# DataArcTech/RAG-ARC

Measured on AMD Instinct MI355X. Metric: queries/sec at fixed (N_corpus, d), exact top-k (ids bit-exact vs CPU oracle), higher is better.
Workload: dtype f16; 1 GPU; 100000000x768 fp16 corpus of N(0,1) directions resident in HBM, row-sharded over 1 GPU(s), batch 256 queries, cosine top-100, exact (canonical fp32 rescore); n_corpus=100000000, d=768, batch=256, k=100, rows_per_gpu=100000000, exchange=none (one shard), repaired_queries_last_step=0

## Files before the change

include/rarc.h:

```cpp
#ifndef RARC_H
#define RARC_H

#include <stddef.h>
#include <stdint.h>

#ifdef __cplusplus
extern "C" {
#endif

#define RARC_VERSION 600

#define RARC_OK 0
#define RARC_E_INVALID -1
#define RARC_E_HIP -2
#define RARC_E_WORKSPACE -3
#define RARC_E_UNSUPPORTED -4
#define RARC_E_IO -5

#define RARC_MAX_QUERIES 256
#define RARC_MAX_K 1024
#define RARC_DIM_ALIGN 128

#define RARC_Q_OK 0u
#define RARC_Q_UNCERTAIN 1u
// ... 231 lines not shown
int rarc_wordpiece_encode(const RarcWordPiece* wp, const char* text_blob, const int64_t* text_offsets, int n_texts,
                          int max_length, int32_t* h_ids, int64_t ld_ids, int32_t* h_lens, int n_threads);

#define RARC_IO_DIRECT 1
#define RARC_IO_FSYNC 2
#define RARC_IO_TRUNCATE 4
typedef struct RarcIoStats {
  int64_t bytes;
  double seconds;
  double file_seconds;
  double copy_wait_seconds;
  int64_t direct_bytes;
  int64_t n_chunks, slot_bytes;
  int n_threads, direct;
} RarcIoStats;
int rarc_file_to_device(const char* path, int n_seg, const int64_t* h_file_off, const int64_t* h_bytes,
                        const int64_t* h_dev_off, void* d_base, int64_t d_capacity_bytes, void* h_staging,
                        size_t staging_bytes, int n_threads, int flags, void* stream, RarcIoStats* stats);
int rarc_device_to_file(const char* path, int n_seg, const int64_t* h_file_off, const int64_t* h_bytes,
                        const int64_t* h_dev_off, const void* d_base, int64_t d_capacity_bytes, void* h_staging,
                        size_t staging_bytes, int n_threads, int flags, void* stream, RarcIoStats* stats);

size_t rarc_wide_workspace_bytes(int d_pad, int cand_cap);
int rarc_search_wide(const void* d_rows, const uint16_t* d_image16, int fmt, int64_t n_rows, int d_pad, float max_norm,
                     float rho, const void* d_qblock, int nq, int k, int64_t id_base, int64_t* d_out_ids,
                     float* d_out_scores, uint32_t* d_status, void* d_ws, size_t ws_bytes, int cand_cap, void* stream);

int rarc_row_sqnorms(const void* d_rows, int fmt, int64_t n_rows, int d_pad, int64_t first_row, float* d_xn, void* stream);
int rarc_search_wide_l2(const void* d_rows, const uint16_t* d_image16, int fmt, int64_t n_rows, int d_pad, float max_norm,
                        float rho, const float* d_xn, const void* d_qblock, int nq, int k, int64_t id_base, int64_t* d_out_ids,
                        float* d_out_scores, uint32_t* d_status, void* d_ws, size_t ws_bytes, int cand_cap, void* stream);
int rarc_debug_wide_bounds(const void* d_ws, size_t ws_bytes, int d_pad, int cand_cap, float* d_out, void* stream);
int rarc_debug_query_scale8(float mx, float* sq, float* qi);

size_t rarc_search_rows_workspace_bytes(int nq, int k);
int rarc_search_rows(const void* d_rows, int fmt, int64_t n_rows, int d_pad, const void* d_qblock, int nq, const int64_t* d_list,
                     int64_t m, int k, int64_t id_base, const float* d_xn, int l2, int64_t* d_out_ids, float* d_out_scores,
                     uint32_t* d_status, void* d_ws, size_t ws_bytes, void* stream);
int rarc_strike_rows(const int64_t* d_ids, const float* d_scores, int nq, int kprime, const uint32_t* d_bits, int64_t n_rows,
                     int64_t id_base, int k, int l2, int64_t* d_out_ids, float* d_out_scores, uint32_t* d_count, void* stream);

size_t rarc_search_rows_grouped_workspace_bytes(int nq, int k);
int rarc_search_rows_grouped(const void* d_rows, int fmt, int64_t n_rows, int d_pad, const void* d_qblock, int nq,
                             const int64_t* d_lists, const int64_t* d_tiles, int n_tiles, int64_t m_max, int k, int64_t id_base,
                             const float* d_xn, int l2, int64_t* d_out_ids, float* d_out_scores, uint32_t* d_status, void* d_ws,
                             size_t ws_bytes, void* stream);
int rarc_strike_rows_grouped(const int64_t* d_ids, const float* d_scores, int nq, int kprime, const uint32_t* d_bits,
                             const int64_t* d_bits_off, int64_t n_rows, int64_t id_base, int k, int l2, int64_t* d_out_ids,
                             float* d_out_scores, uint32_t* d_count, void* stream);

size_t rarc_similar_pairs_workspace_bytes(int64_t n_rows, int d, int cand_cap);
int rarc_similar_pairs(const float* d_rows, int64_t ld, int64_t n_rows, int d, double threshold, void* d_ws, size_t ws_bytes,
                       int cand_cap, int64_t* d_out_pairs, double* d_out_scores, int64_t out_cap,
                       unsigned long long* d_out_count, uint32_t* d_flags, void* stream);

size_t rarc_knn_graph_workspace_bytes(int64_t n_rows, int d, int top_k, int cand_cap);
int rarc_knn_graph(const float* d_rows, int64_t ld, int64_t n_rows, int d, int top_k, double cutoff, void* d_ws, size_t ws_bytes,
                   int cand_cap, int64_t* d_out_ids, double* d_out_scores, int32_t* d_out_count, uint32_t* d_flags, void* stream);

size_t rarc_graph_csr_workspace_bytes(int64_t n, int64_t m);
int rarc_graph_csr(const int64_t* d_pairs, const uint32_t* d_weights, const uint32_t* d_loops, int64_t n, int64_t m, void* d_graph,
                   size_t graph_bytes, void* stream);
size_t rarc_louvain_workspace_bytes(int64_t n, int64_t m);
int rarc_louvain_init(const void* d_graph, size_t graph_bytes, int64_t n, int64_t m, void* d_state, size_t state_bytes, int64_t* d_out3,
                      void* stream);
int rarc_louvain_sweep(const void* d_graph, size_t graph_bytes, int64_t n, int64_t m, void* d_state, size_t state_bytes, int cur, int sweep,
// ... 49 lines not shown
```

rag-arc_amd/csrc/rarc_common.h:

```cpp
#pragma once
#include <hip/hip_runtime.h>
#include <stdint.h>
#include <stddef.h>
#include "../../include/rarc.h"

#if (defined(SCAN_HALFREAD) || defined(RARC_Q8_ABLATIONS) || defined(G256_SKIP_A1)) && !defined(RARC_EXPERIMENT)
#error "SCAN_HALFREAD / RARC_Q8_ABLATIONS / G256_SKIP_A1 build kernels with wrong results: measurement builds only, add -DRARC_EXPERIMENT"
#endif
#ifdef RARC_EXPERIMENT
#define RARC_BUILD_VERSION (RARC_VERSION + 100000)
#else
#define RARC_BUILD_VERSION RARC_VERSION
#endif

typedef _Float16 half_t;
typedef _Float16 half8 __attribute__((ext_vector_type(8)));
typedef float f32x16 __attribute__((ext_vector_type(16)));

#define RARC_GPTR(p) ((const __attribute__((address_space(1))) void*)(p))
#define RARC_LPTR(p) ((__attribute__((address_space(3))) void*)(p))

constexpr int RARC_NB = 256;
constexpr int RARC_MAX_WG = 256;
constexpr int RARC_SEED_TILES = 128;
constexpr int RARC_SEED_MAX_TILES = 2048;
constexpr size_t RARC_WS_THR = 0;
constexpr size_t RARC_WS_BINLO = 1024;
constexpr size_t RARC_WS_BINSCALE = 2048;
constexpr size_t RARC_WS_BININV = 3072;
constexpr size_t RARC_WS_CNT = 4096;
constexpr size_t RARC_WS_FLAGS = 5120;
static_assert(RARC_WS_FLAGS + 4 == RARC_WS_ANYFLAG_OFFSET, "include/rarc.h out of sync");
constexpr size_t RARC_WS_HIST = 8192;
constexpr size_t RARC_WS_CNT2 = RARC_WS_HIST + (size_t)RARC_MAX_QUERIES * RARC_NB * 4;
constexpr size_t RARC_WS_SEED = RARC_WS_CNT2 + (size_t)RARC_MAX_WG * RARC_MAX_QUERIES * 4;
constexpr size_t RARC_WS_CAND = RARC_WS_SEED + (size_t)RARC_MAX_QUERIES * RARC_SEED_MAX_TILES * 32 * 4;

struct RarcWs {
  float* thr;
  float* binlo;
  float* binscale;
  float* bininv;
  uint32_t* cnt;
  uint32_t* flags;
  uint32_t* hist;
  uint32_t* cnt2;
  float* seed;
  uint64_t* cand;
};
static inline RarcWs rarc_ws_carve(void* base) {
  char* b = (char*)base;
  RarcWs w;
  w.thr = (float*)(b + RARC_WS_THR);
  w.binlo = (float*)(b + RARC_WS_BINLO);
  w.binscale = (float*)(b + RARC_WS_BINSCALE);
  w.bininv = (float*)(b + RARC_WS_BININV);
  w.cnt = (uint32_t*)(b + RARC_WS_CNT);
  w.flags = (uint32_t*)(b + RARC_WS_FLAGS);
  w.hist = (uint32_t*)(b + RARC_WS_HIST);
  w.cnt2 = (uint32_t*)(b + RARC_WS_CNT2);
  w.seed = (float*)(b + RARC_WS_SEED);
  w.cand = (uint64_t*)(b + RARC_WS_CAND);
  return w;
}
// ... 263 lines not shown
```

rag-arc_amd/csrc/scan_q8.hip:

```cpp
#include "rarc_common.h"
#include <stdio.h>

struct ScanQ8Params {
  const uint4* corpus;
  const float* tmeta;
  const float* hq;
  const int8_t* q8;
  const float* qinv;
  const float* eps8;
  uint32_t n_rows;
  uint32_t n_tiles;
  uint32_t t_begin;
  uint32_t resume;
  float hot_margin;
  uint32_t* thr;
  const float* binlo;
  const float* binscale;
  const float* bininv;
  uint32_t* hist;
  uint32_t* cnt2;
  uint64_t* cand;
  uint32_t seg;
  uint32_t kprime;
  uint32_t nq;
  unsigned long long* dbg;
};

#ifndef Q8_M16_FP16_ROWS
#define Q8_M16_FP16_ROWS 0
#endif
#ifndef Q8_BIG_PF
#define Q8_BIG_PF 1
#endif
#ifndef Q8_BIG_NG
#define Q8_BIG_NG 2
#endif
#ifndef Q8_EB
#define Q8_EB 0
#endif
constexpr int Q8_WAVES = 8;
constexpr int Q8_THREADS = Q8_WAVES * 64;

constexpr int Q8_WSTAGE = 768;
constexpr int Q8_STAGE = 8 * Q8_WSTAGE;
constexpr int Q8_TB_SLOTS = 16;
constexpr int Q8_TB_STRIDE = 80;

template <bool B>
struct Q8Flag { static constexpr bool value = B; };
constexpr int Q8_DEEP_D = 384;

typedef uint32_t q8_u32x4 __attribute__((ext_vector_type(4)));

template <int D, bool M16V = false>
struct ScanQ8Lds {
  static constexpr int RS = D + (M16V ? 32 : 16);
  static constexpr int TILE = 32 * RS;
  static constexpr int CNT = 2 * TILE;
  static constexpr int BINLO = CNT + 1024;
  static constexpr int BINSCALE = BINLO + 1024;
  static constexpr int BININV = BINSCALE + 1024;
  static constexpr int EPS8 = BININV + 1024;
  static constexpr int HLAND = EPS8 + 1024;
  static constexpr int SKEY = HLAND + 1024;
  static constexpr int SQ = SKEY + 8 * Q8_STAGE;
  static constexpr int TB = (SQ + Q8_STAGE + 15) & ~15;
  static constexpr int TOTAL = TB + Q8_WAVES * Q8_TB_SLOTS * Q8_TB_STRIDE;
};

__device__ __forceinline__ half_t q8_tile_scale(float w) { return __builtin_bit_cast(half_t, (uint16_t)__float_as_uint(w)); }
__device__ __forceinline__ float q8_tile_rt(float w) { return (float)__builtin_bit_cast(half_t, (uint16_t)(__float_as_uint(w) >> 16)); }

__device__ __forceinline__ void q8_lds_barrier() {
  asm volatile("s_waitcnt lgkmcnt(0)\n\ts_barrier" ::: "memory");
}

typedef int q8_i32x16 __attribute__((ext_vector_type(16)));
__device__ __forceinline__ int q8_all16(const q8_i32x16& a) {
  int x = a[0];
#pragma unroll
  for (int i = 1; i < 16; ++i) x ^= a[i];
  return x;
}

template <int D, int FMT = 0, int ABL = 0>
__global__ __launch_bounds__(Q8_THREADS) void rarc_scan_q8_kernel(const ScanQ8Params p) {
  static_assert(D % 128 == 0 && D >= 128 && D <= 1024, "D must be a multiple of 128, <= 1024");
  extern __shared__ __attribute__((aligned(16))) char smem[];
  using L = ScanQ8Lds<D, (FMT != 0) || Q8_M16_FP16_ROWS>;
  constexpr int KS = D / 32;
  static_assert(FMT == 0 || D % 256 == 0, "fp8 rows are padded to a multiple of 256");
  constexpr int EPC = FMT ? 16 : 8;
  constexpr int CPR = D / EPC;
  constexpr int CPT = 32 * CPR / Q8_THREADS;
  constexpr int MSTRIDE = FMT == 1 ? RARC_QMETA_F8_STRIDE : RARC_QMETA_STRIDE;
  constexpr int TCH = 32 * CPR;
  constexpr bool NT_ROWS = !(ABL & 262144);

  const int tid = threadIdx.x;
  const int wave = __builtin_amdgcn_readfirstlane(tid >> 6);
  const int lane = tid & 63;
  const int row = lane & 31, h = lane >> 5;
  constexpr bool M16 = (FMT != 0) || Q8_M16_FP16_ROWS;
  const uint32_t q_lo = wave * 32 + (lane & 15);
  const uint32_t qidx = M16 ? q_lo + 16 * (lane >> 5) : wave * 32 + row;
  const int rq = lane >> 4;
  const int rql = rq & 1;
  auto row_of = [&](uint32_t r) -> uint32_t { return M16 ? (r & 3) + 16 * ((r >> 2) & 1) + 8 * (r >> 3) : (r & 3) + 8 * (r >> 2); };
  const unsigned long long dbg_c0 = p.dbg ? __builtin_amdgcn_s_memtime() : 0ull;
  const unsigned long long dbg_r0 = p.dbg ? __builtin_amdgcn_s_memrealtime() : 0ull;

  uint32_t* s_cnt = (uint32_t*)(smem + L::CNT);
  float* s_binlo = (float*)(smem + L::BINLO);
  float* s_binscale = (float*)(smem + L::BINSCALE);
  float* s_bininv = (float*)(smem + L::BININV);
  float* s_eps8 = (float*)(smem + L::EPS8);
// ... 11 lines not shown

  constexpr int KS2 = D / 64;
  i32x4 qf[KS];
  if constexpr (M16) {
    const int8_t* qp = p.q8 + (size_t)q_lo * D + 16 * rq;
#pragma unroll
    for (int ks = 0; ks < KS2; ++ks) {
      qf[2 * ks] = *(const i32x4*)(qp + 64 * ks);
      qf[2 * ks + 1] = *(const i32x4*)(qp + 16 * D + 64 * ks);
    }
  } else {
    const int8_t* qp = p.q8 + (size_t)qidx * D + 16 * h;
#pragma unroll
    for (int ks = 0; ks < KS; ++ks) qf[ks] = *(const i32x4*)(qp + 32 * ks);
  }
  const float my_qinv = p.qinv[qidx];
  const float my_hq = p.hq[qidx];
  const float r_max = p.tmeta[0 - RARC_QMETA_HDR];
  float thr = __uint_as_float(p.thr[qidx]);
  __builtin_amdgcn_s_waitcnt(0x0F70);

  constexpr bool WOFF_REGS = (D <= 768);
  auto woff_of = [&](int j) {
    const uint32_t c = j * Q8_THREADS + tid;
    return (c / CPR) * L::RS + (c % CPR) * EPC;
  };
  uint32_t woff[WOFF_REGS ? CPT : 1];
  if constexpr (WOFF_REGS) {
#pragma unroll
    for (int j = 0; j < CPT; ++j) woff[j] = woff_of(j);
  }
  const uint32_t aoff = M16 ? (lane & 15) * L::RS + 16 * rq : row * L::RS + 16 * h;

  const uint32_t t0 = p.t_begin + blockIdx.x, stride = gridDim.x;
  const bool has_own = blockIdx.x < p.nq;
  const uint32_t own_q = has_own ? blockIdx.x : 0u;
  const uint32_t* hword = p.hist + (size_t)own_q * RARC_NB + 32 * wave + row;

  struct Fetch {
    uint4 c[CPT];
    float mul[FMT == 1 ? CPT : 1];
    float2 meta;
    uint32_t thr;
    uint32_t hw;
  };
  auto clamp_tile = [&](uint32_t t) { return t < p.n_tiles ? t : 0u; };
  auto fetch = [&](Fetch& f, uint32_t tile, auto refresh) {
    f.meta = *(const float2*)(p.tmeta + (size_t)tile * MSTRIDE);
    if constexpr (FMT == 1) {
#pragma unroll
      for (int j = 0; j < CPT; ++j)
        f.mul[j] = p.tmeta[(size_t)tile * MSTRIDE + 2 + (j * Q8_THREADS + tid) / CPR];
    }
    if constexpr (decltype(refresh)::value) {
      f.thr = __hip_atomic_load(&p.thr[qidx], __ATOMIC_RELAXED, __HIP_MEMORY_SCOPE_AGENT);
      f.hw = __hip_atomic_load(hword, __ATOMIC_RELAXED, __HIP_MEMORY_SCOPE_AGENT);
    }
    __builtin_amdgcn_sched_barrier(0);
    const uint4* src = p.corpus + (size_t)tile * TCH + tid;
#pragma unroll
    for (int j = 0; j < CPT; ++j) {
      if constexpr (NT_ROWS)
        f.c[j] = __builtin_bit_cast(uint4, __builtin_nontemporal_load((const q8_u32x4*)(src + j * Q8_THREADS)));
      else
        f.c[j] = src[j * Q8_THREADS];
    }
  };
  uint32_t opaque_zero = 0;
  asm volatile("" : "+v"(opaque_zero));
  auto convert_chunk = [&](const Fetch& f, int j, half_t s, char* dst) {
    char* at = dst + (WOFF_REGS ? woff[WOFF_REGS ? j : 0] : woff_of(j));
    if constexpr (FMT == 2) {
      const uint4 v = f.c[j];
      *(uint4*)at = make_uint4(v.x ^ opaque_zero, v.y ^ opaque_zero, v.z ^ opaque_zero, v.w ^ opaque_zero);
    } else if constexpr (FMT == 1) {
      if (ABL & 16) {
        const uint4 v = f.c[j];
        *(uint4*)at = make_uint4(v.x ^ opaque_zero, v.y ^ opaque_zero, v.z ^ opaque_zero, v.w ^ opaque_zero);
      } else {
// ... 188 lines not shown
          rs = acc[r] == m ? (uint32_t)r : rs;
        }
      }
      if (__builtin_amdgcn_ballot_w64(c > 1) == 0) {
        const uint32_t doc = row0 + row_of(rs);
        stage_n(pass && doc < p.n_rows, (float)m * sc, doc);
      } else {
#pragma unroll
        for (int r = 0; r < 16; ++r) {
          const float a = (float)acc[r] * sc;
          const uint32_t doc = row0 + row_of((uint32_t)r);
          stage_n(a >= thr && doc < p.n_rows, a, doc);
        }
      }
      }
    }
  };
  auto flush = [&]() __attribute__((always_inline)) {
    drain();
    const uint32_t n = wcount < (uint32_t)Q8_WSTAGE ? wcount : (uint32_t)Q8_WSTAGE;
    for (uint32_t e0 = 0; e0 < n; e0 += 64) {
      const uint32_t e = e0 + lane;
      const bool v = e < n;
      const uint32_t qq = v ? (uint32_t)my_sq[e] : qidx;
      const uint64_t key = v ? my_skey[e] : 0ull;
      const float tcur = __shfl(thr, (int)(M16 ? (qq & 15u) + 2u * (qq & 16u) : (qq & 31u)), 64);
      const bool hot = (ABL & 16384) || rarc_candscore(key) >= tcur + p.hot_margin * s_eps8[qq];
      if (v && rarc_candscore(key) >= tcur) emit(qq, key, hot);
    }
    wcount = 0;
  };

  constexpr int NG = D <= Q8_DEEP_D ? 4 : (FMT != 0 ? (D <= 768 ? 2 : Q8_BIG_NG) : (D <= 896 ? 2 : 1));
  Fetch f[NG];
  fetch(f[0], t0, Q8Flag<true>{});
  convert_tile(f[0], 0);
  float2 mcur[2];
  mcur[0] = f[0].meta;
  __builtin_amdgcn_sched_barrier(0);
  constexpr bool PP = (D <= 768) && !(ABL & 256);
  const bool grp_b = PP && wave >= Q8_WAVES / 2;
  constexpr bool EB = Q8_EB && !PP && !(ABL & 512);
  if constexpr (NG == 4) {
    fetch(f[1], clamp_tile(t0 + stride), Q8Flag<true>{});
    __builtin_amdgcn_sched_barrier(0);
    fetch(f[2], clamp_tile(t0 + 2 * stride), Q8Flag<true>{});
    __builtin_amdgcn_sched_barrier(0);
    fetch(f[3], clamp_tile(t0 + 3 * stride), Q8Flag<true>{});
    __builtin_amdgcn_sched_barrier(0);
    if (!grp_b) fetch(f[0], clamp_tile(t0 + 4 * stride), Q8Flag<true>{});
  } else if constexpr (NG == 2) {
    fetch(f[1], clamp_tile(t0 + stride), Q8Flag<true>{});
    __builtin_amdgcn_sched_barrier(0);
    if (!grp_b) fetch(f[0], clamp_tile(t0 + 2 * stride), Q8Flag<true>{});
  } else {
    fetch(f[0], clamp_tile(t0 + stride), Q8Flag<true>{});
  }
  __builtin_amdgcn_sched_barrier(0);
  float last_pub = has_own ? __uint_as_float(p.thr[own_q]) : -INFINITY;
  __builtin_amdgcn_s_waitcnt(0x0F70);
  q8_lds_barrier();

  i32x16 acc_b = {0};
  bool live_prev = false;
  uint32_t it = 0;
#define Q8_STAMP(slot)                                                                                        \
  if ((ABL & 1024) && blockIdx.x == 0 && it >= 1000 && it < 1016 && lane == 0)                                 \
    p.dbg[8 + ((it - 1000) * Q8_WAVES + wave) * 8 + (slot)] = __builtin_amdgcn_s_memtime();
#define Q8_RF(g) (NG != 4 || (g) == 1)
#define Q8_ITER(PAR, GB, G, GP)                                                                               \
  {                                                                                                           \
    Q8_STAMP(0)                                                                                               \
    if (!(GB)) {             \
      const float tinv = mcur[PAR].y, tsc = mcur[PAR].x;                                                      \
      i32x16 acc;                                                                                             \
      acc = mfma_convert(PAR, f[G]);                                                                  \
      mcur[(PAR) ^ 1] = f[G].meta;                                                                    \
      Q8_STAMP(1)                                                                                             \
      if (!(ABL & 8) && Q8_RF(G)) {                                                                           \
        thr = fmaxf(thr, __uint_as_float(f[G].thr));                                                  \
        if (lane < 32) s_hland[32 * wave + lane] = f[G].hw;                                           \
      }                                                                                                       \
      if constexpr (EB) {                                \
        Q8_STAMP(3)                                                                                           \
        q8_lds_barrier();                                                                                     \
        Q8_STAMP(4)                                                                                           \
      }                                                                                                       \
      if (!(ABL & 1) && live) prune(acc, cur, tinv, tsc);                                                     \
      else if (q8_all16(acc) == 0x7fffffff) p.cnt2[0] = 1;  \
      Q8_STAMP(2)                                                                                             \
                                                                \
      if (!(ABL & 2)) fetch(f[G], clamp_tile(cur + (NG + 1) * stride), Q8Flag<Q8_RF(G)>{});           \
    } else {  \
      if (!(ABL & 1) && live_prev) prune(acc_b, cur - stride, mcur[(PAR) ^ 1].y, mcur[(PAR) ^ 1].x);          \
      live_prev = live;                                                                                       \
      Q8_STAMP(1)                                                                                             \
      if (!(ABL & 2)) fetch(f[GP], clamp_tile(cur + NG * stride), Q8Flag<Q8_RF(GP)>{});                       \
      __builtin_amdgcn_sched_barrier(0);           \
// ... 4 lines not shown
        thr = fmaxf(thr, __uint_as_float(f[G].thr));                                                          \
        if (lane < 32) s_hland[32 * wave + lane] = f[G].hw;                                                   \
      }                                                                                                       \
      if ((ABL & 1) && q8_all16(acc_b) == 0x7fffffff) p.cnt2[0] = 1;                                          \
    }                                                                                                         \
    if constexpr (!EB) {                                                                                      \
      Q8_STAMP(3)                                                                                             \
      q8_lds_barrier();                                                                                       \
      Q8_STAMP(4)                                                                                             \
    }                                                                                                         \
    ++it;                                                                                                     \
                      \
    if (!(ABL & 8) && wave == 0 && has_own && (it <= 16 || (it & 3) == 0)) {                                  \
      const int b = rarc_wave_find_from_top_256(s_hland[4 * lane], s_hland[4 * lane + 1],                     \
                                                s_hland[4 * lane + 2], s_hland[4 * lane + 3], p.kprime);      \
      if (b >= 2 && lane == 0) {                                                                              \
        const float lo = s_binlo[own_q];                                                                      \
        const float t = fmaxf(rarc_bin_threshold(b, lo, s_bininv[own_q]) - 2.0002f * s_eps8[own_q], lo);      \
        if (t > last_pub) {                  \
          last_pub = t;                                                                                       \
          __hip_atomic_store(&p.thr[own_q], __float_as_uint(t), __ATOMIC_RELAXED, __HIP_MEMORY_SCOPE_AGENT);  \
        }                                                                                                     \
      }                                                                                                       \
    }                                                                                                         \
                  \
    if (!(ABL & 64) && (wcount | tb_n) != 0 &&                                                                 \
        (it <= 16 || (it & (it - 1)) == 0 || (it & 127) == 0 || wcount > (uint32_t)Q8_WSTAGE / 2))            \
      flush();                                                                                                \
  }

#define Q8_STEP(OFF, PAR, GB, G, GP)                                                  \
    {                                                                                 \
      const uint32_t cur = base + (OFF) * stride;                                     \
      const bool live = (OFF) == 0 || cur < p.n_tiles;                                \
      Q8_ITER(PAR, GB, G, GP)                                                         \
    }
#define Q8_LOOP(GB)                                                                   \
  if constexpr (NG == 4) {                                                            \
    for (uint32_t base = t0; base < p.n_tiles; base += 4 * stride) {                  \
      Q8_STEP(0, 0, GB, 1, 0) Q8_STEP(1, 1, GB, 2, 1) Q8_STEP(2, 0, GB, 3, 2) Q8_STEP(3, 1, GB, 0, 3) \
    }                                                                                 \
  } else {                                                                            \
    for (uint32_t base = t0; base < p.n_tiles; base += 2 * stride) {                  \
      Q8_STEP(0, 0, GB, NG == 2 ? 1 : 0, 0) Q8_STEP(1, 1, GB, 0, NG == 2 ? 1 : 0)     \
    }                                                                                 \
  }
  if (grp_b) {
    Q8_LOOP(true)
  } else {
    Q8_LOOP(false)
  }
#undef Q8_STEP
#undef Q8_LOOP
#undef Q8_ITER
#undef Q8_RF
  if (grp_b && !(ABL & 1) && live_prev)
    prune(acc_b, t0 + (((p.n_tiles - 1 - t0) / stride) | (NG == 4 ? 3u : 1u)) * stride, mcur[1].y, mcur[1].x);
  flush();
  __syncthreads();
  if (tid < RARC_MAX_QUERIES) p.cnt2[(size_t)blockIdx.x * RARC_MAX_QUERIES + tid] = s_cnt[tid];
  if (p.dbg && blockIdx.x == 0 && tid == 0) {
    p.dbg[0] = __builtin_amdgcn_s_memtime() - dbg_c0;
    p.dbg[1] = __builtin_amdgcn_s_memrealtime() - dbg_r0;
  }
}

bool rarc_prof_next(hipEvent_t* start, hipEvent_t* stop);
int rarc_seed_launch(const void* corpus, const float* rowscale, int fmt, int64_t n_rows, int d_pad,
                     const uint16_t* q16, int nq, int kprime, float bin_lo, float bin_hi, const float* sub_a,
                     const float* sub_b, const RarcWs& ws, hipStream_t s, int64_t rows_covered, const float* floor);
int rarc_scan_f16_stage_launch(const uint16_t* corpus, int64_t n_rows, uint32_t stage_tiles, int d_pad, const uint16_t* q16,
                               const float* eps16, int nq, int kprime, const RarcWs& ws, int cap, int grid, hipStream_t s);

template <int D, int FMT, int ABL = 0>
static int launch_scan_q8(const ScanQ8Params& p, int grid, hipStream_t s) {
  constexpr size_t lds = ScanQ8Lds<D, (FMT != 0) || Q8_M16_FP16_ROWS>::TOTAL;
  static RarcPerDevice attr_done;
  if (size_t& done = attr_done.cur(); !done) {
    RARC_HIP_CHECK(hipFuncSetAttribute((const void*)rarc_scan_q8_kernel<D, FMT, ABL>,
                                       hipFuncAttributeMaxDynamicSharedMemorySize, (int)lds));
    done = 1;
  }
#ifdef RARC_Q8_ABLATIONS
  if constexpr (ABL == 0 && ((D == 1024 && FMT == 1) || (D == 768 && FMT == 0) || (D == 768 && FMT == 2))) {
    static const int abl = getenv("RARC_Q8_ABL") ? atoi(getenv("RARC_Q8_ABL")) : 0;
    if (abl == 262144) return launch_scan_q8<D, FMT, 262144>(p, grid, s);
    if (abl == 262149) return launch_scan_q8<D, FMT, 262149>(p, grid, s);
    if (abl == 1) return launch_scan_q8<D, FMT, 1>(p, grid, s);
    if (abl == 4) return launch_scan_q8<D, FMT, 4>(p, grid, s);
    if (abl == 5) return launch_scan_q8<D, FMT, 5>(p, grid, s);
    if (abl == 9) return launch_scan_q8<D, FMT, 9>(p, grid, s);
    if constexpr (FMT == 1) {
      if (abl == 1024 || abl == 1025) {
        static unsigned long long* d_dbg = nullptr;
        if (!d_dbg) RARC_HIP_CHECK(hipMalloc((void**)&d_dbg, 65536));
        RARC_HIP_CHECK(hipMemsetAsync(d_dbg, 0, 65536, s));
        ScanQ8Params pd = p;
        pd.dbg = d_dbg;
        hipFuncSetAttribute((const void*)rarc_scan_q8_kernel<D, FMT, 1024>, hipFuncAttributeMaxDynamicSharedMemorySize, (int)lds);
        hipFuncSetAttribute((const void*)rarc_scan_q8_kernel<D, FMT, 1025>, hipFuncAttributeMaxDynamicSharedMemorySize, (int)lds);
        if (abl == 1024) hipLaunchKernelGGL((rarc_scan_q8_kernel<D, FMT, 1024>), dim3(grid), dim3(Q8_THREADS), lds, s, pd);
        else hipLaunchKernelGGL((rarc_scan_q8_kernel<D, FMT, 1025>), dim3(grid), dim3(Q8_THREADS), lds, s, pd);
        RARC_HIP_CHECK(hipStreamSynchronize(s));
        if (const char* path = getenv("RARC_Q8_TIMELINE"); path && p.n_tiles - p.t_begin > 1100u * (uint32_t)grid) {
          static unsigned long long h[8192];
          RARC_HIP_CHECK(hipMemcpy(h, d_dbg, 65536, hipMemcpyDeviceToHost));
          if (FILE* f = fopen(path, "a")) {
            fprintf(f, "launch tiles [%u, %u) abl %d: per iteration and wave, shader cycles relative to wave 0's start of the iteration: start | after mfma+convert | after prune | after fetch issue | after barrier\n", p.t_begin, p.n_tiles, abl);
            for (int it = 2; it < 10; ++it)
              for (int w = 0; w < Q8_WAVES; ++w) {
                const unsigned long long* r = &h[8 + (it * Q8_WAVES + w) * 8];
                const unsigned long long b0 = h[8 + (it * Q8_WAVES) * 8];
                fprintf(f, "it %2d w%d: %6lld %6lld %6lld %6lld %6lld   (next iteration starts at %lld)\n", it, w, (long long)(r[0] - b0), (long long)(r[1] - b0),
                        (long long)(r[2] - b0), (long long)(r[3] - b0), (long long)(r[4] - b0), (long long)(h[8 + ((it + 1) * Q8_WAVES + w) * 8] - b0));
              }
            fclose(f);
          }
        }
// ... 41 lines not shown
                 FMTV == 0 ? 128 : 256);
  return RARC_E_UNSUPPORTED;
}

int rarc_scan_q8_launch(const void* corpus, const float* rowscale, int fmt, int64_t n_rows, int d_pad,
                        const float* qmeta, const uint16_t* q16, const int8_t* q8, const float* qinv,
                        const float* eps16, const float* eps8, int nq, int kprime, float bin_lo, float bin_hi,
                        const RarcWs& ws, int cap, int* grid_out, hipStream_t s, const int8_t* shadow8,
                        int (*tighten)(void* ctx, int n_wg, int mode), void* tighten_ctx, const float* hq, const float* floor,
                        int* hybrid_out) {
  ScanQ8Params p;
  p.hq = hq;
  p.corpus = fmt == 2 ? (const uint4*)shadow8 : (const uint4*)corpus;
  p.tmeta = qmeta + RARC_QMETA_HDR;
  p.q8 = q8;
  p.qinv = qinv;
  p.eps8 = eps8;
  p.n_rows = (uint32_t)n_rows;
  p.n_tiles = (uint32_t)((n_rows + 31) / 32);
  p.t_begin = 0;
  p.resume = 0;
  p.hot_margin = 1.0f;
  p.thr = (uint32_t*)ws.thr;
  p.binlo = ws.binlo;
  p.binscale = ws.binscale;
  p.bininv = ws.bininv;
  p.hist = ws.hist;
  p.cnt2 = ws.cnt2;
  p.cand = ws.cand;
  p.seg = (uint32_t)(cap / RARC_MAX_WG);
  p.kprime = (uint32_t)kprime;
  p.nq = (uint32_t)nq;
  p.dbg = nullptr;

  int dev = 0, cus = 256;
  RARC_HIP_CHECK(hipGetDevice(&dev));
  RARC_HIP_CHECK(hipDeviceGetAttribute(&cus, hipDeviceAttributeMultiprocessorCount, dev));
  int grid = cus < RARC_MAX_WG ? cus : RARC_MAX_WG;
  if (const char* e = getenv("RARC_SCAN_Q8_WGS")) { const int g = atoi(e); if (g >= 8 && g < grid) grid = g; }
  if ((uint32_t)grid > p.n_tiles) grid = (int)p.n_tiles;
  *grid_out = grid;
  auto launch = [&](const ScanQ8Params& pp) {
    return fmt == 2 ? dispatch_scan_q8<2>(pp, d_pad, grid, s)
                    : fmt == 1 ? dispatch_scan_q8<1>(pp, d_pad, grid, s) : dispatch_scan_q8<0>(pp, d_pad, grid, s);
  };
  static const int split_mode = getenv("RARC_SCAN_SPLIT") ? atoi(getenv("RARC_SCAN_SPLIT")) : 3;
  const uint32_t pair = 2u * (uint32_t)(grid > 0 ? grid : 1);
  uint32_t cuts[3];
  int n_cuts = 0;
  if (tighten && split_mode > 0) {
    uint32_t div[3] = {512u, 64u, 8u};
    if (const char* e = getenv("RARC_SPLIT_DIVS")) {
      unsigned a = 0, b = 0, c = 0;
      const int got = sscanf(e, "%u,%u,%u", &a, &b, &c);
      if (got >= 1) { div[0] = a; div[1] = got >= 2 ? b : 0; div[2] = got >= 3 ? c : 0; }
    }
    for (int i = (split_mode >= 3 ? 0 : (split_mode == 2 ? 1 : 2)); i < 3; ++i) {
      if (div[i] == 0) continue;
      const uint32_t t = (p.n_tiles / div[i]) / pair * pair;
      static const int min_env = getenv("RARC_SPLIT_MIN") ? atoi(getenv("RARC_SPLIT_MIN")) : 0;
      const uint32_t min_pairs = min_env > 0 ? (uint32_t)min_env : (div[i] == 8u ? 16u : 8u);
      if (t >= min_pairs * pair && (n_cuts == 0 || t > cuts[n_cuts - 1])) cuts[n_cuts++] = t;
    }
  }
  int rc = rarc_seed_launch(corpus, rowscale, fmt == 2 ? 0 : fmt, n_rows, d_pad, q16, nq, kprime, bin_lo, bin_hi, eps16,
                            eps8, ws, s, n_cuts ? (int64_t)cuts[0] * 32 : 0, floor);
  if (rc) return rc;
  if (p.n_tiles == 0) return RARC_OK;
  RARC_REQUIRE(rarc_gate_scan(s) == 0, RARC_E_HIP, "rarc_scan_q8: hipStreamWaitEvent on the gate event failed");
  uint32_t begin = 0;
  static const int hybrid_env = getenv("RARC_HYBRID") ? atoi(getenv("RARC_HYBRID")) : 1;
  static const int hybrid_div = getenv("RARC_HYBRID_DIV") ? atoi(getenv("RARC_HYBRID_DIV")) : 8;
  if (hybrid_out) *hybrid_out = 0;
  if (hybrid_out && hybrid_env && tighten && fmt == 0 && d_pad <= 768 && n_cuts == 0 && hybrid_div >= 2) {
    const uint32_t stage = (p.n_tiles / (uint32_t)hybrid_div) / pair * pair;
    if (stage >= 2u * pair && stage < p.n_tiles) {
      if ((rc = rarc_scan_f16_stage_launch((const uint16_t*)corpus, n_rows, stage, d_pad, q16, eps16, nq, kprime, ws, cap, grid,
                                           s)) != RARC_OK)
        return rc;
      if ((rc = tighten(tighten_ctx, grid, 2)) != RARC_OK) return rc;
      ScanQ8Params pi = p;
      pi.t_begin = stage;
      pi.resume = 1u;
      pi.hot_margin = 0.f;
      *hybrid_out = 1;
      return launch(pi);
    }
  }
  for (int i = 0; i <= n_cuts; ++i) {
    ScanQ8Params pi = p;
    pi.t_begin = begin;
    pi.n_tiles = i < n_cuts ? cuts[i] : p.n_tiles;
    pi.resume = i > 0 ? 1u : 0u;
    pi.hot_margin = i > 0 ? 0.f : 1.0f;
    if ((rc = launch(pi)) != RARC_OK) return rc;
    if (i < n_cuts && (rc = tighten(tighten_ctx, grid, 1)) != RARC_OK) return rc;
    begin = pi.n_tiles;
  }
  return RARC_OK;
}
```

rag-arc_amd/hip/binding.py:

```python
from __future__ import annotations

import ctypes
import os
import threading
from ctypes import c_double, c_float, c_int, c_int64, c_size_t, c_uint64, c_void_p

_PKG = os.path.dirname(os.path.dirname(os.path.abspath(__file__)))
_LIB = os.environ.get("RARC_LIBRARY") or os.path.join(_PKG, "lib", "librarc_hip.so")

MAX_QUERIES = 256
MAX_K = 1024
WIDE_MAX_K = 8192
WIDE_MAX_DPAD = 4096
DIM_ALIGN = 128
Q_UNCERTAIN = 1
Q_OVERFLOW = 2
WS_ANYFLAG_OFFSET = 5124


class RarcError(RuntimeError):
    """Raised for every non-zero status returned by librarc_hip.so."""


class RarcUnsupported(RarcError, NotImplementedError):
# ... 140 lines not shown
    "rarc_enc32_gemm": (c_int, [c_void_p, c_void_p, c_void_p, c_void_p, c_void_p, c_void_p, c_int, c_int, c_int, c_void_p]),
    "rarc_enc32_workspace_bytes": (c_size_t, [c_int, c_int, c_int]),
    "rarc_enc32_forward": (c_int, [c_void_p, c_void_p, c_void_p, c_int, c_int, c_int, c_void_p, c_size_t, c_void_p,
                                   c_void_p]),
    "rarc_lm_workspace_bytes": (c_size_t, [c_void_p, c_int]),
    "rarc_lm_yes_no_logits": (c_int, [c_void_p, c_void_p, c_void_p, c_int, c_int, c_int, c_int, c_void_p, c_size_t, c_void_p,
                                      c_void_p]),
    "rarc_lm_prefix_cache_bytes": (c_size_t, [c_void_p, c_int]),
    "rarc_lm_prefix_kv": (c_int, [c_void_p, c_void_p, c_void_p, c_int, c_int, c_void_p, c_size_t, c_void_p, c_size_t, c_void_p]),
    "rarc_lm_yes_no_logits_prefixed": (c_int, [c_void_p, c_void_p, c_void_p, c_int, c_int, c_void_p, c_void_p, c_int, c_int,
                                                c_void_p, c_int, c_int, c_void_p, c_size_t, c_void_p, c_void_p]),
    "rarc_lm_embed_last": (c_int, [c_void_p, c_void_p, c_void_p, c_int, c_int, c_int, c_int, c_void_p, c_size_t, c_void_p, c_int64,
                                   c_void_p]),
    "rarc_lm_embed_last_prefixed": (c_int, [c_void_p, c_void_p, c_void_p, c_int, c_int, c_void_p, c_void_p, c_int, c_int, c_void_p,
                                            c_int, c_int, c_void_p, c_size_t, c_void_p, c_int64, c_void_p]),
    "rarc_wordpiece_create": (c_int, [ctypes.c_char_p, c_size_t, c_int, ctypes.c_char_p, ctypes.c_char_p, ctypes.c_char_p,
                                      ctypes.c_char_p, ctypes.c_char_p, c_size_t, c_int, ctypes.POINTER(c_void_p)]),
    "rarc_wordpiece_destroy": (None, [c_void_p]),
    "rarc_wordpiece_encode": (c_int, [c_void_p, ctypes.c_char_p, c_void_p, c_int, c_int, c_void_p, c_int64, c_void_p, c_int]),
    "rarc_file_to_device": (c_int, [ctypes.c_char_p, c_int, ctypes.POINTER(c_int64), ctypes.POINTER(c_int64),
                                    ctypes.POINTER(c_int64), c_void_p, c_int64, c_void_p, c_size_t, c_int, c_int, c_void_p,
                                    ctypes.POINTER(IoStats)]),
    "rarc_device_to_file": (c_int, [ctypes.c_char_p, c_int, ctypes.POINTER(c_int64), ctypes.POINTER(c_int64),
                                    ctypes.POINTER(c_int64), c_void_p, c_int64, c_void_p, c_size_t, c_int, c_int, c_void_p,
                                    ctypes.POINTER(IoStats)]),
    "rarc_wide_workspace_bytes": (c_size_t, [c_int, c_int]),
    "rarc_search_wide": (c_int, [c_void_p, c_void_p, c_int, c_int64, c_int, c_float, c_float, c_void_p, c_int, c_int, c_int64,
                                 c_void_p, c_void_p, c_void_p, c_void_p, c_size_t, c_int, c_void_p]),
    "rarc_row_sqnorms": (c_int, [c_void_p, c_int, c_int64, c_int, c_int64, c_void_p, c_void_p]),
    "rarc_search_wide_l2": (c_int, [c_void_p, c_void_p, c_int, c_int64, c_int, c_float, c_float, c_void_p, c_void_p, c_int, c_int,
                                    c_int64, c_void_p, c_void_p, c_void_p, c_void_p, c_size_t, c_int, c_void_p]),
    "rarc_debug_wide_bounds": (c_int, [c_void_p, c_size_t, c_int, c_int, c_void_p, c_void_p]),
    "rarc_debug_query_scale8": (c_int, [c_float, ctypes.POINTER(c_float), ctypes.POINTER(c_float)]),
    "rarc_search_rows_workspace_bytes": (c_size_t, [c_int, c_int]),
    "rarc_search_rows": (c_int, [c_void_p, c_int, c_int64, c_int, c_void_p, c_int, c_void_p, c_int64, c_int, c_int64, c_void_p, c_int,
                                 c_void_p, c_void_p, c_void_p, c_void_p, c_size_t, c_void_p]),
    "rarc_strike_rows": (c_int, [c_void_p, c_void_p, c_int, c_int, c_void_p, c_int64, c_int64, c_int, c_int, c_void_p, c_void_p,
                                 c_void_p, c_void_p]),
    "rarc_search_rows_grouped_workspace_bytes": (c_size_t, [c_int, c_int]),
    "rarc_search_rows_grouped": (c_int, [c_void_p, c_int, c_int64, c_int, c_void_p, c_int, c_void_p, c_void_p, c_int, c_int64, c_int,
                                         c_int64, c_void_p, c_int, c_void_p, c_void_p, c_void_p, c_void_p, c_size_t, c_void_p]),
    "rarc_strike_rows_grouped": (c_int, [c_void_p, c_void_p, c_int, c_int, c_void_p, c_void_p, c_int64, c_int64, c_int, c_int,
                                         c_void_p, c_void_p, c_void_p, c_void_p]),
    "rarc_similar_pairs_workspace_bytes": (c_size_t, [c_int64, c_int, c_int]),
    "rarc_similar_pairs": (c_int, [c_void_p, c_int64, c_int64, c_int, ctypes.c_double, c_void_p, c_size_t, c_int, c_void_p, c_void_p,
                                   c_int64, c_void_p, c_void_p, c_void_p]),
    "rarc_knn_graph_workspace_bytes": (c_size_t, [c_int64, c_int, c_int, c_int]),
    "rarc_knn_graph": (c_int, [c_void_p, c_int64, c_int64, c_int, c_int, ctypes.c_double, c_void_p, c_size_t, c_int, c_void_p, c_void_p,
                               c_void_p, c_void_p, c_void_p]),
    "rarc_graph_csr_workspace_bytes": (c_size_t, [c_int64, c_int64]),
    "rarc_graph_csr": (c_int, [c_void_p, c_void_p, c_void_p, c_int64, c_int64, c_void_p, c_size_t, c_void_p]),
    "rarc_louvain_workspace_bytes": (c_size_t, [c_int64, c_int64]),
    "rarc_louvain_init": (c_int, [c_void_p, c_size_t, c_int64, c_int64, c_void_p, c_size_t, c_void_p, c_void_p]),
    "rarc_louvain_sweep": (c_int, [c_void_p, c_size_t, c_int64, c_int64, c_void_p, c_size_t, c_int, c_int, c_void_p, c_void_p]),
    "rarc_louvain_aggregate": (c_int, [c_void_p, c_size_t, c_int64, c_int64, c_void_p, c_size_t, c_int, c_void_p, c_int64, c_void_p,
                                       c_void_p, c_void_p, c_void_p, c_void_p]),
    "rarc_louvain_labels_workspace_bytes": (c_size_t, [c_int64]),
    "rarc_louvain_labels": (c_int, [c_void_p, c_int64, c_void_p, c_size_t, c_void_p]),
    "rarc_louvain_limits": (c_int, [ctypes.POINTER(c_int)]),
    "rarc_ppr_workspace_bytes": (c_size_t, [c_int64, c_int64, c_int]),
    "rarc_ppr_seed": (c_int, [c_void_p, c_size_t, c_int64, c_int64, c_void_p, c_void_p, c_int, c_int, c_void_p, c_size_t, c_void_p]),
    "rarc_ppr_step": (c_int, [c_void_p, c_size_t, c_int64, c_int64, c_int, c_int, c_int64, c_int, c_void_p, c_size_t, c_void_p,
                              c_void_p]),
    "rarc_ppr_scores": (c_int, [c_int64, c_int64, c_int, c_void_p, c_size_t, c_void_p, c_void_p]),
    "rarc_ppr_topk": (c_int, [c_int64, c_int64, c_int, c_int, c_int, c_void_p, c_size_t, c_void_p, c_void_p, c_void_p, c_void_p]),
    "rarc_ppr_limits": (c_int, [ctypes.POINTER(c_int)]),
# ... 59 lines not shown
```

Before: 9480 queries/s.

## Add dynamic tail scheduling with guided chunk claims to q8 scan

```diff
diff --git a/include/rarc.h b/include/rarc.h
--- a/include/rarc.h
+++ b/include/rarc.h
@@ -287,6 +287,11 @@
                         float* d_out_scores, uint32_t* d_status, void* d_ws, size_t ws_bytes, int cand_cap, void* stream);
 int rarc_debug_wide_bounds(const void* d_ws, size_t ws_bytes, int d_pad, int cand_cap, float* d_out, void* stream);
 int rarc_debug_query_scale8(float mx, float* sq, float* qi);
+int rarc_debug_q8_tail_plan(uint32_t t_begin, uint32_t n_tiles, uint32_t grid, int d_pad, int fmt, int pct, int min_mib,
+                            uint32_t* t_dyn, uint32_t* r0, uint32_t* unit);
+int rarc_debug_q8_tail_chunks(uint32_t k_first, uint32_t n, uint32_t stride, uint32_t unit, uint32_t t_dyn, uint32_t r0,
+                              uint32_t n_tiles, uint32_t* t0, uint32_t* t_end);
+int64_t rarc_debug_q8_tail_counter_offset(int launch);
 
 size_t rarc_search_rows_workspace_bytes(int nq, int k);
 int rarc_search_rows(const void* d_rows, int fmt, int64_t n_rows, int d_pad, const void* d_qblock, int nq, const int64_t* d_list,
diff --git a/rag-arc_amd/csrc/rarc_common.h b/rag-arc_amd/csrc/rarc_common.h
--- a/rag-arc_amd/csrc/rarc_common.h
+++ b/rag-arc_amd/csrc/rarc_common.h
@@ -30,6 +30,7 @@
 constexpr size_t RARC_WS_BININV = 3072;
 constexpr size_t RARC_WS_CNT = 4096;
 constexpr size_t RARC_WS_FLAGS = 5120;
+constexpr int RARC_WS_TAIL_FLAG = 32;
 static_assert(RARC_WS_FLAGS + 4 == RARC_WS_ANYFLAG_OFFSET, "include/rarc.h out of sync");
 constexpr size_t RARC_WS_HIST = 8192;
 constexpr size_t RARC_WS_CNT2 = RARC_WS_HIST + (size_t)RARC_MAX_QUERIES * RARC_NB * 4;
diff --git a/rag-arc_amd/csrc/scan_q8.hip b/rag-arc_amd/csrc/scan_q8.hip
--- a/rag-arc_amd/csrc/scan_q8.hip
+++ b/rag-arc_amd/csrc/scan_q8.hip
@@ -1,5 +1,8 @@
 #include "rarc_common.h"
 #include <stdio.h>
+#ifdef RARC_Q8_ABLATIONS
+#include <algorithm>
+#endif
 
 struct ScanQ8Params {
   const uint4* corpus;
@@ -23,6 +26,9 @@
   uint32_t seg;
   uint32_t kprime;
   uint32_t nq;
+  uint32_t t_dyn;
+  uint32_t tail_r0;
+  uint32_t* tail_ctr;
   unsigned long long* dbg;
 };
 
@@ -45,6 +51,9 @@
 constexpr int Q8_STAGE = 8 * Q8_WSTAGE;
 constexpr int Q8_TB_SLOTS = 16;
 constexpr int Q8_TB_STRIDE = 80;
+constexpr int Q8_DBG_BYTES = 65536;
+constexpr int Q8_FIN_SLOT = 2048;
+static_assert((Q8_FIN_SLOT + 2 * RARC_MAX_WG) * 8 <= Q8_DBG_BYTES, "finish stamps past the debug buffer");
 
 template <bool B>
 struct Q8Flag { static constexpr bool value = B; };
@@ -65,7 +74,8 @@
   static constexpr int SKEY = HLAND + 1024;
   static constexpr int SQ = SKEY + 8 * Q8_STAGE;
   static constexpr int TB = (SQ + Q8_STAGE + 15) & ~15;
-  static constexpr int TOTAL = TB + Q8_WAVES * Q8_TB_SLOTS * Q8_TB_STRIDE;
+  static constexpr int TICK = TB + Q8_WAVES * Q8_TB_SLOTS * Q8_TB_STRIDE;
+  static constexpr int TOTAL = TICK + 16;
 };
 
 __device__ __forceinline__ half_t q8_tile_scale(float w) { return __builtin_bit_cast(half_t, (uint16_t)__float_as_uint(w)); }
@@ -82,6 +92,39 @@
   for (int i = 1; i < 16; ++i) x ^= a[i];
   return x;
 }
+
+constexpr uint32_t Q8_TAIL_RMIN = 8;
+__host__ __device__ inline void q8_tail_chunk(uint32_t k, uint32_t stride, uint32_t unit, uint32_t t_dyn, uint32_t r0,
+                                              uint32_t n_tiles, uint32_t* t0, uint32_t* t_end) {
+  const uint32_t level = k / stride, slot = k - level * stride;
+  uint32_t r = r0 < Q8_TAIL_RMIN ? Q8_TAIL_RMIN : r0, start = 0;
+  for (uint32_t i = 0; i < level && (uint64_t)t_dyn + (uint64_t)start * stride < n_tiles; ++i) {
+    start += r;
+    r = (r >> 1) / unit * unit;
+    if (r < Q8_TAIL_RMIN) r = Q8_TAIL_RMIN;
+  }
+  const uint64_t first = (uint64_t)t_dyn + (uint64_t)start * stride + slot, end = (uint64_t)t_dyn + (uint64_t)(start + r) * stride;
+  *t0 = first < n_tiles ? (uint32_t)first : n_tiles;
+  *t_end = end < n_tiles ? (uint32_t)end : n_tiles;
+}
+
+inline bool q8_tail_plan(uint32_t t_begin, uint32_t n_tiles, uint32_t g, uint32_t unit, uint32_t pct, uint64_t tile_bytes,
+                         uint64_t min_bytes, uint32_t* t_dyn, uint32_t* r0) {
+  *t_dyn = n_tiles;
+  *r0 = 0;
+  if (g == 0 || unit == 0 || n_tiles <= t_begin) return false;
+  const uint32_t rounds = (uint32_t)(((uint64_t)(n_tiles - t_begin) + g - 1) / g);
+  const uint32_t share = (uint32_t)((uint64_t)rounds * (pct > 100u ? 100u : pct) / 100u);
+  if (share < unit || (uint64_t)rounds * tile_bytes < min_bytes) return false;
+  uint32_t stat = (rounds - share) / unit * unit;
+  if (stat < unit) stat = unit;
+  const uint64_t td = (uint64_t)t_begin + (uint64_t)stat * g;
+  if (td >= n_tiles) return false;
+  *t_dyn = (uint32_t)td;
+  *r0 = (uint32_t)((((uint64_t)(n_tiles - *t_dyn) + g - 1) / g / 2) / unit * unit);
+  return true;
+}
+inline uint32_t q8_tail_unit(int d_pad) { return d_pad <= 384 ? 4u : 2u; }
 
 template <int D, int FMT = 0, int ABL = 0>
 __global__ __launch_bounds__(Q8_THREADS) void rarc_scan_q8_kernel(const ScanQ8Params p) {
@@ -159,7 +202,8 @@
   }
   const uint32_t aoff = M16 ? (lane & 15) * L::RS + 16 * rq : row * L::RS + 16 * h;
 
-  const uint32_t t0 = p.t_begin + blockIdx.x, stride = gridDim.x;
+  const uint32_t stride = gridDim.x;
+  uint32_t t0 = p.t_begin + blockIdx.x, t_end = p.tail_ctr ? p.t_dyn : p.n_tiles;
   const bool has_own = blockIdx.x < p.nq;
   const uint32_t own_q = has_own ? blockIdx.x : 0u;
   const uint32_t* hword = p.hist + (size_t)own_q * RARC_NB + 32 * wave + row;
@@ -171,7 +215,7 @@
     uint32_t thr;
     uint32_t hw;
   };
-  auto clamp_tile = [&](uint32_t t) { return t < p.n_tiles ? t : 0u; };
+  auto clamp_tile = [&](uint32_t t) { return t < t_end ? t : 0u; };
   auto fetch = [&](Fetch& f, uint32_t tile, auto refresh) {
     f.meta = *(const float2*)(p.tmeta + (size_t)tile * MSTRIDE);
     if constexpr (FMT == 1) {
@@ -426,6 +470,9 @@
   };
 
   constexpr int NG = D <= Q8_DEEP_D ? 4 : (FMT != 0 ? (D <= 768 ? 2 : Q8_BIG_NG) : (D <= 896 ? 2 : 1));
+  float last_pub = has_own ? __uint_as_float(p.thr[own_q]) : -INFINITY;
+  uint32_t it = 0;
+  do {
   Fetch f[NG];
   fetch(f[0], t0, Q8Flag<true>{});
   convert_tile(f[0], 0);
@@ -451,13 +498,11 @@
     fetch(f[0], clamp_tile(t0 + stride), Q8Flag<true>{});
   }
   __builtin_amdgcn_sched_barrier(0);
-  float last_pub = has_own ? __uint_as_float(p.thr[own_q]) : -INFINITY;
   __builtin_amdgcn_s_waitcnt(0x0F70);
   q8_lds_barrier();
 
   i32x16 acc_b = {0};
   bool live_prev = false;
-  uint32_t it = 0;
 #define Q8_STAMP(slot)                                                                                        \
   if ((ABL & 1024) && blockIdx.x == 0 && it >= 1000 && it < 1016 && lane == 0)                                 \
     p.dbg[8 + ((it - 1000) * Q8_WAVES + wave) * 8 + (slot)] = __builtin_amdgcn_s_memtime();
@@ -528,16 +573,16 @@
 #define Q8_STEP(OFF, PAR, GB, G, GP)                                                  \
     {                                                                                 \
       const uint32_t cur = base + (OFF) * stride;                                     \
-      const bool live = (OFF) == 0 || cur < p.n_tiles;                                \
+      const bool live = (OFF) == 0 || cur < t_end;                                \
       Q8_ITER(PAR, GB, G, GP)                                                         \
     }
 #define Q8_LOOP(GB)                                                                   \
   if constexpr (NG == 4) {                                                            \
-    for (uint32_t base = t0; base < p.n_tiles; base += 4 * stride) {                  \
+    for (uint32_t base = t0; base < t_end; base += 4 * stride) {                  \
       Q8_STEP(0, 0, GB, 1, 0) Q8_STEP(1, 1, GB, 2, 1) Q8_STEP(2, 0, GB, 3, 2) Q8_STEP(3, 1, GB, 0, 3) \
     }                                                                                 \
   } else {                                                                            \
-    for (uint32_t base = t0; base < p.n_tiles; base += 2 * stride) {                  \
+    for (uint32_t base = t0; base < t_end; base += 2 * stride) {                  \
       Q8_STEP(0, 0, GB, NG == 2 ? 1 : 0, 0) Q8_STEP(1, 1, GB, 0, NG == 2 ? 1 : 0)     \
     }                                                                                 \
   }
@@ -551,7 +596,16 @@
 #undef Q8_ITER
 #undef Q8_RF
   if (grp_b && !(ABL & 1) && live_prev)
-    prune(acc_b, t0 + (((p.n_tiles - 1 - t0) / stride) | (NG == 4 ? 3u : 1u)) * stride, mcur[1].y, mcur[1].x);
+    prune(acc_b, t0 + (((t_end - 1 - t0) / stride) | (NG == 4 ? 3u : 1u)) * stride, mcur[1].y, mcur[1].x);
+  t0 = p.n_tiles;
+  if (p.tail_ctr) {
+    uint32_t* s_tick = (uint32_t*)(smem + L::TICK);
+    if (tid == 0) *s_tick = atomicAdd(p.tail_ctr, 1u);
+    __syncthreads();
+    const uint32_t k = __builtin_amdgcn_readfirstlane(*s_tick);
+    q8_tail_chunk(k, stride, NG == 4 ? 4u : 2u, p.t_dyn, p.tail_r0, p.n_tiles, &t0, &t_end);
+  }
+  } while (t0 < p.n_tiles);
   flush();
   __syncthreads();
   if (tid < RARC_MAX_QUERIES) p.cnt2[(size_t)blockIdx.x * RARC_MAX_QUERIES + tid] = s_cnt[tid];
@@ -559,6 +613,13 @@
     p.dbg[0] = __builtin_amdgcn_s_memtime() - dbg_c0;
     p.dbg[1] = __builtin_amdgcn_s_memrealtime() - dbg_r0;
   }
+#ifdef RARC_Q8_ABLATIONS
+  if (!(ABL & 1024) && p.dbg && tid == 0) {
+    __builtin_amdgcn_s_waitcnt(0x0F70);
+    p.dbg[Q8_FIN_SLOT + 2 * blockIdx.x] = dbg_r0;
+    p.dbg[Q8_FIN_SLOT + 2 * blockIdx.x + 1] = __builtin_amdgcn_s_memrealtime();
+  }
+#endif
 }
 
 bool rarc_prof_next(hipEvent_t* start, hipEvent_t* stop);
@@ -567,6 +628,56 @@
                      const float* sub_b, const RarcWs& ws, hipStream_t s, int64_t rows_covered, const float* floor);
 int rarc_scan_f16_stage_launch(const uint16_t* corpus, int64_t n_rows, uint32_t stage_tiles, int d_pad, const uint16_t* q16,
                                const float* eps16, int nq, int kprime, const RarcWs& ws, int cap, int grid, hipStream_t s);
+
+#ifdef RARC_Q8_ABLATIONS
+template <int D, int FMT>
+static int launch_scan_q8_finish(const ScanQ8Params& p, int grid, hipStream_t s, const char* path) {
+  constexpr size_t lds = ScanQ8Lds<D, (FMT != 0) || Q8_M16_FP16_ROWS>::TOTAL;
+  static unsigned long long* d_dbg = nullptr;
+  if (!d_dbg) RARC_HIP_CHECK(hipMalloc((void**)&d_dbg, Q8_DBG_BYTES));
+  RARC_REQUIRE(grid >= 1 && grid <= RARC_MAX_WG, RARC_E_HIP, "launch_scan_q8_finish: grid %d", grid);
+  RARC_HIP_CHECK(hipMemsetAsync(d_dbg, 0, Q8_DBG_BYTES, s));
+  ScanQ8Params pd = p;
+  pd.dbg = d_dbg;
+  hipEvent_t e0, e1;
+  const bool prof = rarc_prof_next(&e0, &e1);
+  if (prof) RARC_HIP_CHECK(hipEventRecord(e0, s));
+  hipLaunchKernelGGL((rarc_scan_q8_kernel<D, FMT, 0>), dim3(grid), dim3(Q8_THREADS), lds, s, pd);
+  RARC_HIP_CHECK(hipGetLastError());
+  if (prof) RARC_HIP_CHECK(hipEventRecord(e1, s));
+  RARC_HIP_CHECK(hipStreamSynchronize(s));
+  static unsigned long long h[2 * RARC_MAX_WG];
+  RARC_HIP_CHECK(hipMemcpy(h, d_dbg + Q8_FIN_SLOT, sizeof(unsigned long long) * 2 * grid, hipMemcpyDeviceToHost));
+  FILE* f = fopen(path, "a");
+  if (!f) return RARC_OK;
+  double st[RARC_MAX_WG], en[RARC_MAX_WG];
+  unsigned long long s0 = ~0ull;
+  for (int b = 0; b < grid; ++b) s0 = h[2 * b] < s0 ? h[2 * b] : s0;
+  for (int b = 0; b < grid; ++b) { st[b] = (double)(h[2 * b] - s0) * 0.01; en[b] = (double)(h[2 * b + 1] - s0) * 0.01; }
+  auto median = [](double* v, int n) { std::sort(v, v + n); return n ? 0.5 * (v[(n - 1) / 2] + v[n / 2]) : 0.0; };
+  double xs[8], xe[8];
+  for (int x = 0; x < 8; ++x) {
+    double a[RARC_MAX_WG / 8 + 1], e[RARC_MAX_WG / 8 + 1];
+    int n = 0;
+    for (int b = x; b < grid; b += 8, ++n) { a[n] = st[b]; e[n] = en[b]; }
+    xs[x] = median(a, n);
+    xe[x] = median(e, n);
+  }
+  double mean = 0;
+  for (int b = 0; b < grid; ++b) mean += en[b] / grid;
+  std::sort(st, st + grid);
+  const double med = median(en, grid), first = en[0], last = en[grid - 1], len = last;
+  fprintf(f, "launch tiles [%u, %u) grid %d: %.1f us | ends: last-first %.1f us (%.2f %%) last-median %.1f us (%.2f %%) last-mean %.1f us (%.2f %%)"
+          " | starts: last-first %.1f us | per XCD median end - first end:", p.t_begin, p.n_tiles, grid, len, last - first,
+          100 * (last - first) / len, last - med, 100 * (last - med) / len, last - mean, 100 * (last - mean) / len, st[grid - 1]);
+  for (int x = 0; x < 8; ++x) fprintf(f, " %.1f", xe[x] - first);
+  fprintf(f, " | per XCD median start:");
+  for (int x = 0; x < 8; ++x) fprintf(f, " %.1f", xs[x]);
+  fprintf(f, "\n");
+  fclose(f);
+  return RARC_OK;
+}
+#endif
 
 template <int D, int FMT, int ABL = 0>
 static int launch_scan_q8(const ScanQ8Params& p, int grid, hipStream_t s) {
@@ -580,6 +691,8 @@
 #ifdef RARC_Q8_ABLATIONS
   if constexpr (ABL == 0 && ((D == 1024 && FMT == 1) || (D == 768 && FMT == 0) || (D == 768 && FMT == 2))) {
     static const int abl = getenv("RARC_Q8_ABL") ? atoi(getenv("RARC_Q8_ABL")) : 0;
+    if (abl == 0)
+      if (const char* path = getenv("RARC_Q8_FINISH")) return launch_scan_q8_finish<D, FMT>(p, grid, s, path);
     if (abl == 262144) return launch_scan_q8<D, FMT, 262144>(p, grid, s);
     if (abl == 262149) return launch_scan_q8<D, FMT, 262149>(p, grid, s);
     if (abl == 1) return launch_scan_q8<D, FMT, 1>(p, grid, s);
@@ -687,6 +800,9 @@
   p.kprime = (uint32_t)kprime;
   p.nq = (uint32_t)nq;
   p.dbg = nullptr;
+  p.t_dyn = p.n_tiles;
+  p.tail_r0 = 0;
+  p.tail_ctr = nullptr;
 
   int dev = 0, cus = 256;
   RARC_HIP_CHECK(hipGetDevice(&dev));
@@ -698,6 +814,18 @@
   auto launch = [&](const ScanQ8Params& pp) {
     return fmt == 2 ? dispatch_scan_q8<2>(pp, d_pad, grid, s)
                     : fmt == 1 ? dispatch_scan_q8<1>(pp, d_pad, grid, s) : dispatch_scan_q8<0>(pp, d_pad, grid, s);
+  };
+  int tail_pct = 16;
+  if (const char* e = getenv("RARC_SCAN_Q8_TAIL")) tail_pct = atoi(e);
+  tail_pct = tail_pct < 0 ? 0 : (tail_pct > 100 ? 100 : tail_pct);
+  int tail_min_mib = 32;
+  if (const char* e = getenv("RARC_SCAN_Q8_TAIL_MIN")) tail_min_mib = atoi(e);
+  const uint64_t tile_bytes = 32ull * (uint64_t)d_pad * (fmt == 0 ? 2u : 1u);
+  static_assert(Q8_DEEP_D == 384, "q8_tail_unit");
+  auto set_tail = [&](ScanQ8Params& pp, int launch_idx) {
+    const bool tail = q8_tail_plan(pp.t_begin, pp.n_tiles, (uint32_t)grid, q8_tail_unit(d_pad), (uint32_t)tail_pct, tile_bytes,
+                                   (uint64_t)(tail_min_mib > 0 ? tail_min_mib : 0) << 20, &pp.t_dyn, &pp.tail_r0);
+    pp.tail_ctr = tail ? ws.flags + RARC_WS_TAIL_FLAG + launch_idx : nullptr;
   };
   static const int split_mode = getenv("RARC_SCAN_SPLIT") ? atoi(getenv("RARC_SCAN_SPLIT")) : 3;
   const uint32_t pair = 2u * (uint32_t)(grid > 0 ? grid : 1);
@@ -739,6 +867,7 @@
       pi.resume = 1u;
       pi.hot_margin = 0.f;
       *hybrid_out = 1;
+      set_tail(pi, 0);
       return launch(pi);
     }
   }
@@ -748,9 +877,29 @@
     pi.n_tiles = i < n_cuts ? cuts[i] : p.n_tiles;
     pi.resume = i > 0 ? 1u : 0u;
     pi.hot_margin = i > 0 ? 0.f : 1.0f;
+    set_tail(pi, i);
     if ((rc = launch(pi)) != RARC_OK) return rc;
     if (i < n_cuts && (rc = tighten(tighten_ctx, grid, 1)) != RARC_OK) return rc;
     begin = pi.n_tiles;
   }
   return RARC_OK;
 }
+
+extern "C" int rarc_debug_q8_tail_plan(uint32_t t_begin, uint32_t n_tiles, uint32_t grid, int d_pad, int fmt, int pct, int min_mib,
+                                       uint32_t* t_dyn, uint32_t* r0, uint32_t* unit) {
+  RARC_REQUIRE(t_dyn && r0 && unit, RARC_E_INVALID, "rarc_debug_q8_tail_plan: null pointer");
+  RARC_REQUIRE(d_pad > 0 && fmt >= 0 && fmt <= 2, RARC_E_INVALID, "rarc_debug_q8_tail_plan: d_pad %d, row format %d", d_pad, fmt);
+  *unit = q8_tail_unit(d_pad);
+  q8_tail_plan(t_begin, n_tiles, grid, *unit, (uint32_t)(pct < 0 ? 0 : pct), 32ull * (uint64_t)d_pad * (fmt == 0 ? 2u : 1u),
+               (uint64_t)(min_mib > 0 ? min_mib : 0) << 20, t_dyn, r0);
+  return RARC_OK;
+}
+extern "C" int rarc_debug_q8_tail_chunks(uint32_t k_first, uint32_t n, uint32_t stride, uint32_t unit, uint32_t t_dyn, uint32_t r0,
+                                         uint32_t n_tiles, uint32_t* t0, uint32_t* t_end) {
+  RARC_REQUIRE(t0 && t_end && stride > 0 && unit > 0, RARC_E_INVALID, "rarc_debug_q8_tail_chunks: null pointer, stride or unit 0");
+  for (uint32_t i = 0; i < n; ++i) q8_tail_chunk(k_first + i, stride, unit, t_dyn, r0, n_tiles, &t0[i], &t_end[i]);
+  return RARC_OK;
+}
+extern "C" int64_t rarc_debug_q8_tail_counter_offset(int launch) {
+  return launch >= 0 && launch < 4 ? (int64_t)(RARC_WS_FLAGS + 4 * (size_t)(RARC_WS_TAIL_FLAG + launch)) : -1;
+}
diff --git a/rag-arc_amd/hip/binding.py b/rag-arc_amd/hip/binding.py
--- a/rag-arc_amd/hip/binding.py
+++ b/rag-arc_amd/hip/binding.py
@@ -196,6 +196,10 @@
                                     c_int64, c_void_p, c_void_p, c_void_p, c_void_p, c_size_t, c_int, c_void_p]),
     "rarc_debug_wide_bounds": (c_int, [c_void_p, c_size_t, c_int, c_int, c_void_p, c_void_p]),
     "rarc_debug_query_scale8": (c_int, [c_float, ctypes.POINTER(c_float), ctypes.POINTER(c_float)]),
+    "rarc_debug_q8_tail_plan": (c_int, [ctypes.c_uint32, ctypes.c_uint32, ctypes.c_uint32, c_int, c_int, c_int, c_int,
+                                        ctypes.POINTER(ctypes.c_uint32), ctypes.POINTER(ctypes.c_uint32), ctypes.POINTER(ctypes.c_uint32)]),
+    "rarc_debug_q8_tail_chunks": (c_int, [ctypes.c_uint32] * 7 + [c_void_p, c_void_p]),
+    "rarc_debug_q8_tail_counter_offset": (c_int64, [c_int]),
     "rarc_search_rows_workspace_bytes": (c_size_t, [c_int, c_int]),
     "rarc_search_rows": (c_int, [c_void_p, c_int, c_int64, c_int, c_void_p, c_int, c_void_p, c_int64, c_int, c_int64, c_void_p, c_int,
                                  c_void_p, c_void_p, c_void_p, c_void_p, c_size_t, c_void_p]),
```

New measurement: 9664 queries/s, median of 6. 1.02x the previous value.
